# derekc22/UR3e

Measured on NVIDIA B200. Metric: env-steps/sec (UR3e+2F85, physics+controller), higher is better.
Workload: dtype f32

## Files before the change

ur3e_b200/csrc/batch_impl.cuh:

```cuda
#pragma once
#include <cstdio>
#include <cstdlib>
#include <cstring>
#include <limits>
#include <type_traits>
#include <vector>

#include "batch_base.h"
#include "compile_model.h"
#include "merge_bodies.h"
#include "env.cuh"
#include "query.cuh"
#include "query_fwd.cuh"
#include "render.cuh"
#include "rollout.h"

#ifndef UR3E_BLOCKS_PER_SM
#define UR3E_BLOCKS_PER_SM 2
#endif
#ifndef UR3E_LS_TOL
#define UR3E_LS_TOL 1e-2
#endif
#ifndef UR3E_MAX_WPB
#define UR3E_MAX_WPB 16
#endif

namespace ur3e {
enum Op { OP_STEP = 0, OP_RESET = 1, OP_SET_STATE = 2 };

template <typename Real>
struct KArgs {
  const DevModel<Real>* m;
  EnvCfg<Real> c;
  SolverOpts<Real> opt;
  const EnvCfg<Real>* c_dev; const SolverOpts<Real>* opt_dev;
  void* st;
  int* ovf_count; int* ovf_list;
  const int* list_count; const int* list;
  int lite_maxcon, lite_maxefc;
  int mid_maxcon, mid_maxefc;
  int* ovf2_count; int* ovf2_list;
  int* ovf_stat;
  int cap_con, cap_efc;
  long long n;
  int op;
  const Real* act; Real* obs; Real* rew; uint8_t* term; uint8_t* trunc; Real* final_obs;
  Real* sens;
  const uint8_t* mask;
  unsigned long long seed, env_base;
  const Real* qpos_in; const Real* qvel_in; const Real* ws_in;
};

template <typename Real, typename D> __host__ __device__ constexpr size_t arena_stride() { return (sizeof(Arena<Real, D>) + 15) / 16 * 16; }
template <typename Real, typename D> __host__ __device__ constexpr int warps_per_block() {
#ifdef UR3E_FORCE_WPB
  return UR3E_FORCE_WPB;
#endif
  int per_sm = (int)((233472 - 1024 * UR3E_BLOCKS_PER_SM) / arena_stride<Real, D>());
  int w = per_sm / UR3E_BLOCKS_PER_SM;
#ifdef UR3E_MID_MAX_WPB
  if (D::EXACT && D::MAXCON == 16 && w > UR3E_MID_MAX_WPB) w = UR3E_MID_MAX_WPB;
#endif
  return w > UR3E_MAX_WPB ? UR3E_MAX_WPB : (w < 1 ? 1 : w);
}

template <typename Real, typename D>
__global__ void __launch_bounds__(warps_per_block<Real, D>() * 32) env_kernel(const KArgs<Real> a) {
  constexpr int WPB = warps_per_block<Real, D>();
  extern __shared__ int4 smem_raw[];
  const int warp = threadIdx.x >> 5;
  const long long e = (long long)blockIdx.x * WPB + warp;
  if (e >= a.n) return;
  Arena<Real, D>& s = *reinterpret_cast<Arena<Real, D>*>(reinterpret_cast<unsigned char*>(smem_raw) + warp * arena_stride<Real, D>());
  const DevModel<Real>& m = *a.m;
  const EnvCfg<Real>& c = a.c;
  constexpr int NW = sizeof(EnvState<Real, D>) / 16;
  int4* gst = reinterpret_cast<int4*>(static_cast<EnvState<Real, D>*>(a.st) + e);
  int4* sst = reinterpret_cast<int4*>(&s.st);
  if (a.op == OP_RESET && a.mask && !a.mask[e]) return;
  WARP_FOR(i, NW) sst[i] = gst[i];
  IF_LANE0 { s.overflow = 0; s.ncon = 0; s.nefc = 0; s.solver_iter = 0; s.cap_con = D::MAXCON; s.cap_efc = D::MAXEFC; }
  WARP_SYNC();
  const int od = c.obs_dim;
  IF_LANE0 s.st.tier = 0;
  if (a.op == OP_RESET) {
    env_reset(m, c, s, a.opt, a.seed, a.env_base + (unsigned long long)e);
    ContactFlags cf = contact_flags(m, c, s);
    write_obs(m, c, s, cf);
    if (a.obs) { WARP_FOR(i, od) a.obs[e * od + i] = s.obs[i]; }
  } else if (a.op == OP_SET_STATE) {
    WARP_FOR(i, m.nq) s.st.qpos[i] = a.qpos_in[e * m.nq + i];
    WARP_FOR(i, m.nv) { s.st.qvel[i] = a.qvel_in[e * m.nv + i]; s.st.qacc_ws[i] = a.ws_in ? a.ws_in[e * m.nv + i] : Real(0); }
    WARP_SYNC();
    forward_cold(m, s, a.opt, false);
    update_cache(m, c, s);
  }
  WARP_SYNC();
  WARP_FOR(i, NW) gst[i] = sst[i];
}

constexpr int TIER_HOLD = 8;
template <typename Real, typename D, bool SENS = false>
__global__ void __launch_bounds__(warps_per_block<Real, D>() * 32, UR3E_BLOCKS_PER_SM) step_kernel(const KArgs<Real> a) {
  constexpr int WPB = warps_per_block<Real, D>();
  extern __shared__ int4 smem_raw[];
  const int warp = threadIdx.x >> 5;
  Arena<Real, D>& s = *reinterpret_cast<Arena<Real, D>*>(reinterpret_cast<unsigned char*>(smem_raw) + warp * arena_stride<Real, D>());
  const DevModel<Real>& m = *a.m;
  const EnvCfg<Real>& c = a.c;
  constexpr int NW = sizeof(EnvState<Real, D>) / 16;
  const int od = c.obs_dim;
  long long count = a.n; int iters = 1;
  if (a.list) { count = *a.list_count; const long long per = (long long)gridDim.x * WPB; iters = (int)((count + per - 1) / per); }
  for (int it = 0; it < iters; ++it) {
    const long long idx = ((long long)it * gridDim.x + blockIdx.x) * WPB + warp;
    if (idx >= count) return;
    const long long e = a.list ? (long long)a.list[idx] : idx;
    EnvState<Real, D>* const rec = static_cast<EnvState<Real, D>*>(a.st) + e;
    if (a.ovf_list && !a.list) {
      const int tier = rec->tier;
      if (tier & 0xff) {
        IF_LANE0 {
          if ((tier >> 8) && a.ovf2_list) { const int k = atomicAdd(a.ovf2_count, 1); a.ovf2_list[k] = (int)e; }
          else { const int k = atomicAdd(a.ovf_count, 1); a.ovf_list[k] = (int)e; }
        }
        return;
      }
    }
    int4* gst = reinterpret_cast<int4*>(rec);
    int4* sst = reinterpret_cast<int4*>(&s.st);
    WARP_FOR(i, NW) sst[i] = gst[i];
    IF_LANE0 {
      s.overflow = 0; s.ncon = 0; s.nefc = 0; s.solver_iter = 0;
      s.cap_con = (a.cap_con > 0 && a.cap_con < D::MAXCON) ? a.cap_con : D::MAXCON; s.cap_efc = (a.cap_efc > 0 && a.cap_efc < D::MAXEFC) ? a.cap_efc : D::MAXEFC;
    }
    WARP_SYNC();
    StepOut<Real> r = env_step(m, c, s, a.opt, a.act + e * c.act_dim, *a.opt_dev, SENS ? a.sens : nullptr, e);
    if (a.ovf_list && s.overflow) {
      IF_LANE0 { const int k = atomicAdd(a.ovf_count, 1); a.ovf_list[k] = (int)e; }
      continue;
    }
    if (a.lite_maxcon > 0) {
      IF_LANE0 {
        const bool big = s.max_ncon > a.lite_maxcon || s.max_nefc > a.lite_maxefc;
        const bool big2 = a.mid_maxcon > 0 && (s.max_ncon > a.mid_maxcon || s.max_nefc > a.mid_maxefc);
        const int h1 = s.st.tier & 0xff, h2 = s.st.tier >> 8;
        s.st.tier = (big ? TIER_HOLD : (h1 > 0 ? h1 - 1 : 0)) | ((big2 ? TIER_HOLD : (h2 > 0 ? h2 - 1 : 0)) << 8);
        if (big && a.ovf_stat) atomicAdd(a.ovf_stat, 1);
      }
    }
    const int done = r.terminated | r.truncated;
    if (done && a.final_obs) { WARP_FOR(i, od) a.final_obs[e * od + i] = s.obs[i]; }
    if (done && c.auto_reset) {
      env_reset(m, *a.c_dev, s, *a.opt_dev, a.seed, a.env_base + (unsigned long long)e);
      ContactFlags cf = contact_flags(m, c, s);
      write_obs(m, c, s, cf);
    }
    WARP_FOR(i, od) a.obs[e * od + i] = s.obs[i];
    IF_LANE0 { a.rew[e] = r.reward; a.term[e] = (uint8_t)r.terminated; a.trunc[e] = (uint8_t)r.truncated; }
    WARP_SYNC();
    WARP_FOR(i, NW) gst[i] = sst[i];
    WARP_SYNC();
  }
}

template <typename Real, typename D>
__global__ void state_io_kernel(EnvState<Real, D>* st, long long n, int nq, int nv, Real* qpos, Real* qvel, Real* ws) {
  long long i = (long long)blockIdx.x * blockDim.x + threadIdx.x;
  long long e = i / 64; int k = (int)(i % 64);
  if (e >= n) return;
  if (k < nq && qpos) qpos[e * nq + k] = st[e].qpos[k];
  if (k < nv && qvel) qvel[e * nv + k] = st[e].qvel[k];
  if (k < nv && ws) ws[e * nv + k] = st[e].qacc_ws[k];
}

template <typename Real, typename D>
__global__ void stats_kernel(EnvState<Real, D>* st, long long n, double* out, int reset) {
  long long e = (long long)blockIdx.x * blockDim.x + threadIdx.x;
  for (int k = 0; k < NSTAT; ++k) {
    double d = 0.0;
    if (e < n) { d = k == ST_RETURN ? (double)st[e].stat[k].f : (double)st[e].stat[k].i; if (reset) st[e].stat[k].i = 0; }
    for (int o = 16; o > 0; o >>= 1) d += __shfl_xor_sync(0xffffffffu, d, o);
    if ((threadIdx.x & 31) == 0 && d != 0.0) atomicAdd(out + k, d);
  }
}

template <typename Real, typename D>
__global__ void rollout_gather_kernel(const EnvState<Real, D>* src, long long n, const int* ids, EnvState<Real, D>* dst, long long m) {
  const long long j = ((long long)blockIdx.x * blockDim.x + threadIdx.x) >> 5;
  const int lane = threadIdx.x & 31;
  if (j >= m) return;
  constexpr int NW = sizeof(EnvState<Real, D>) / 16;
  const long long e = ids[j];
  int4* d = reinterpret_cast<int4*>(dst + j);
  const bool valid = e >= 0 && e < n;
  if (valid) {
    const int4* g = reinterpret_cast<const int4*>(src + e);
    for (int i = lane; i < NW; i += 32) d[i] = g[i];
  } else {
    for (int i = lane; i < NW; i += 32) d[i] = make_int4(0, 0, 0, 0);
  }
  __syncwarp();
  EnvState<Real, D>& r = dst[j];
  if (valid) {
    if (lane < NSTAT) r.stat[lane].i = 0;
  } else {
    const Real nan = std::numeric_limits<Real>::quiet_NaN();
    for (int i = lane; i < D::NQ; i += 32) r.qpos[i] = nan;
    for (int i = lane; i < D::NV; i += 32) { r.qvel[i] = nan; r.qacc_ws[i] = nan; }
    for (int i = lane; i < CACHE_SIZE; i += 32) r.cache[i] = nan;
  }
}

template <typename Real, typename D>
// ... 29 lines not shown
  WARP_SYNC();
  const long long k = a.k;
  query_env(m, s, a.q, a.k, a.pos ? a.pos + e * k * 3 : nullptr, a.mat ? a.mat + e * k * 9 : nullptr, a.vel ? a.vel + e * k * 6 : nullptr, a.local);
}

template <typename Real, typename D>
struct QJArgs {
  const DevModel<Real>* m;
  const EnvState<Real, D>* st;
  const QueryEntry<Real>* q; int k;
  long long n;
  Real *jacp, *jacr, *M, *bias;
};

template <typename Real, typename D>
__global__ void __launch_bounds__(warps_per_block<Real, QueryDims<D>>() * 32) query_jac_kernel(const QJArgs<Real, D> a) {
  using DK = QueryDims<D>;
  constexpr int WPB = warps_per_block<Real, DK>();
  extern __shared__ int4 smem_raw[];
  const int warp = threadIdx.x >> 5;
  const long long e = (long long)blockIdx.x * WPB + warp;
  if (e >= a.n) return;
  Arena<Real, DK>& s = *reinterpret_cast<Arena<Real, DK>*>(reinterpret_cast<unsigned char*>(smem_raw) + warp * arena_stride<Real, DK>());
  const DevModel<Real>& m = *a.m;
  const EnvState<Real, D>& rec = a.st[e];
  WARP_FOR(i, m.nq) s.st.qpos[i] = rec.qpos[i];
  if (a.M || a.bias) { WARP_FOR(i, m.nv) s.st.qvel[i] = rec.qvel[i]; }
  WARP_SYNC();
  const long long nv = m.nv, kj = (long long)a.k * 3 * nv;
  query_jac_env(m, s, a.q, a.k, a.jacp ? a.jacp + e * kj : nullptr, a.jacr ? a.jacr + e * kj : nullptr, a.M ? a.M + e * nv * nv : nullptr,
                a.bias ? a.bias + e * nv : nullptr);
}

template <typename Real, typename D>
struct QFArgs {
  const DevModel<Real>* m;
  const EnvState<Real, D>* st;
  SolverOpts<Real> opt;
  long long n;
  const Real* ctrl;
  FwdOut<Real> o;
};

template <typename Real, typename D>
__global__ void __launch_bounds__(warps_per_block<Real, D>() * 32, 1) query_fwd_kernel(const QFArgs<Real, D> a) {
  constexpr int WPB = warps_per_block<Real, D>();
  constexpr long long C = D::HAS_CONTACT ? D::MAXCON : 0;
  extern __shared__ int4 smem_raw[];
  const int warp = threadIdx.x >> 5;
  const long long e = (long long)blockIdx.x * WPB + warp;
  if (e >= a.n) return;
  Arena<Real, D>& s = *reinterpret_cast<Arena<Real, D>*>(reinterpret_cast<unsigned char*>(smem_raw) + warp * arena_stride<Real, D>());
  const DevModel<Real>& m = *a.m;
  constexpr int NW = sizeof(EnvState<Real, D>) / 16;
  const int4* gst = reinterpret_cast<const int4*>(a.st + e);
  int4* sst = reinterpret_cast<int4*>(&s.st);
  WARP_FOR(i, NW) sst[i] = gst[i];
  const long long nv = m.nv;
  FwdOut<Real> o;
  o.qacc = a.o.qacc ? a.o.qacc + e * nv : nullptr;
  o.qfrc_constraint = a.o.qfrc_constraint ? a.o.qfrc_constraint + e * nv : nullptr;
  o.info = a.o.info ? a.o.info + e * 4 : nullptr;
  o.contact_geom = a.o.contact_geom ? a.o.contact_geom + e * C * 2 : nullptr;
  o.contact_dist = a.o.contact_dist ? a.o.contact_dist + e * C : nullptr;
  o.contact_pos = a.o.contact_pos ? a.o.contact_pos + e * C * 3 : nullptr;
  o.contact_frame = a.o.contact_frame ? a.o.contact_frame + e * C * 9 : nullptr;
  o.contact_force = a.o.contact_force ? a.o.contact_force + e * C * 6 : nullptr;
  o.flags = a.o.flags ? a.o.flags + e : nullptr;
  o.sensordata = a.o.sensordata ? a.o.sensordata + e * NSENSOR : nullptr;
  forward_query_env(m, s, a.opt, a.ctrl ? a.ctrl + e * m.nu : nullptr, o);
}

template <typename Real, typename D>
struct RPArgs {
  const DevModel<Real>* m;
  const EnvState<Real, D>* st;
  const QueryEntry<Real>* q; int k;
  long long n, count;
  const int* env_ids;
  Real* pose;
};

template <typename Real, typename D>
__global__ void __launch_bounds__(warps_per_block<Real, QueryDims<D>>() * 32) render_pose_kernel(const RPArgs<Real, D> a) {
  using DK = QueryDims<D>;
  constexpr int WPB = warps_per_block<Real, DK>();
  extern __shared__ int4 smem_raw[];
  const int warp = threadIdx.x >> 5;
  const long long i = (long long)blockIdx.x * WPB + warp;
  if (i >= a.count) return;
  const long long e = a.env_ids ? (long long)a.env_ids[i] : i;
  if (e < 0 || e >= a.n) return;
  Arena<Real, DK>& s = *reinterpret_cast<Arena<Real, DK>*>(reinterpret_cast<unsigned char*>(smem_raw) + warp * arena_stride<Real, DK>());
  const DevModel<Real>& m = *a.m;
  const EnvState<Real, D>& rec = a.st[e];
  WARP_FOR(j, m.nq) s.st.qpos[j] = rec.qpos[j];
  WARP_SYNC();
  render_pose_env(m, s, a.q, a.k, a.pose + i * 12 * (a.k + 1));
}

template <typename Real>
struct RArgs {
  const RenderGeom<Real>* geoms; int k;
  RenderCam<Real> cam;
  const Real* pose;
  const int* env_ids; long long n;
  unsigned char* rgb; Real* depth; int* seg;
};

constexpr int RENDER_THREADS = 256, RENDER_TILE = 1024;
// ... 493 lines not shown
```

ur3e_b200/csrc/engine.cuh:

```cuda
#pragma once
#include "dev_model.h"
#include "warp_model.cuh"

namespace ur3e {

template <int NB_, int NV_, int NQ_, int NU_, int NG_, int NPAIR_, int MAXCON_, int MAXEFC_, int SPLIT_ = NV_, bool EXACT_ = false>
struct Dims {
  static constexpr bool EXACT = EXACT_;
  static constexpr int SPLIT = SPLIT_;
  static constexpr int NB = NB_, NV = NV_, NQ = NQ_, NU = NU_, NG = NG_ > 0 ? NG_ : 1, NPAIR = NPAIR_ > 0 ? NPAIR_ : 1;
  static constexpr int MAXCON = MAXCON_ > 0 ? MAXCON_ : 1, MAXEFC = MAXEFC_ > 0 ? MAXEFC_ : 1;
  static constexpr bool HAS_CONTACT = MAXCON_ > 0;
  static constexpr int NS = MAXSITE;
  static constexpr int ACT_CAP = MAXCON_ <= 8 ? 16 : (MAXCON_ <= 16 ? 20 : 24);
  static constexpr int MAXACT = !HAS_CONTACT ? 1 : (NPAIR < ACT_CAP ? NPAIR : ACT_CAP);
  static constexpr int NGRP = MAXEQ + (NPAIR < MAXCON ? NPAIR : MAXCON);
  static constexpr int MAXCONNECT = 2;
  static constexpr int MAXDENSE = HAS_CONTACT ? 3 * MAXCONNECT + 3 * MAXCON : 1;
};
using DimsRaw = Dims<8, 6, 6, 6, 1, 0, 0, 12>;
using DimsGrip = Dims<17, 14, 14, 7, 6, 12, 12, 56>;
using DimsGripExact = Dims<17, 14, 14, 7, 6, 12, 12, 56, 14, true>;
using DimsMain = Dims<19, 20, 21, 7, 14, 48, 24, 92, 14>;
using DimsMainLite = Dims<19, 20, 21, 7, 14, 48, 8, 44, 14, true>;
using DimsMainMid = Dims<19, 20, 21, 7, 14, 48, 16, 68, 14, true>;

constexpr int STAGE_PTS = 8;
constexpr int STAGE_W = 3 + 4 * STAGE_PTS;

enum RowType { ROW_EQ = 0, ROW_EQJ = 1, ROW_FRICTION = 2, ROW_LIMIT_LO = 3, ROW_LIMIT_HI = 4, ROW_CON_N = 5, ROW_CON_T1 = 6, ROW_CON_T2 = 7 };

constexpr int NSTAT = 16;
constexpr int MAX_FRAME_SKIP = 256;
enum StatSlot { ST_EPISODES = 0, ST_RETURN, ST_LENGTH, ST_SUCCESS, ST_TERM_REACH, ST_TERM_TOPPLE, ST_TERM_COLLISION, ST_TRUNC, ST_UNSTABLE,
                ST_NEFC, ST_NCON, ST_ITER, ST_SUBSTEPS, ST_OVERFLOW,
                ST_PADCON , ST_STEPS  };
template <typename Real, typename D>
struct alignas(16) EnvState {
  Real qpos[D::NQ], qvel[D::NV], qacc_ws[D::NV];
  Real cache[CACHE_SIZE];
  Real ep_return;
  union { int i; float f; } stat[NSTAT];
  int t, episode;
  int tier;
};

#ifdef UR3E_CANARY
#define UR3E_GUARD(n) unsigned guard##n;
constexpr unsigned CANARY_WORD = 0xC0FFEE5Au;
#else
#define UR3E_GUARD(n)
#endif

template <typename Real, typename D>
struct Arena {
  EnvState<Real, D> st;
  UR3E_GUARD(0)
  Real qacc[D::NV], ctrl[D::NU], act_force[D::NU];
  Real xpos[D::NB][3];
  union alignas(8) {
    struct { Real xmat[D::NB][9], xipos[D::NB][3]; } k;
    struct { Real H[(D::NV + 1) * (D::NV + 2) / 2]; } n;
  } fr;
  union { alignas(16) Real colbuf[1][32]; Real obs[32]; };
  Real cdof[D::NV][6];
  UR3E_GUARD(1)
  alignas(8) Real M[D::NV * (D::NV + 1) / 2];
  UR3E_GUARD(2)
  Real qfrc_smooth[D::NV], qfrc_bias[D::NV], qfrc_constraint[D::NV], grad[D::NV], search[D::NV], Ma[D::NV];
  union { Real Mv[D::NV]; Real dinv[D::NV]; };
  Real site_xpos[D::NS][3], site_xmat[1][9] , site_velp[D::NS][3];
  Real con_pos[D::MAXCON][3], con_dist[D::MAXCON], con_mu[D::MAXCON];
  union {
    Real frame[D::MAXCON][9];
    Real gpos[D::NG][3];
  } cu;
  static_assert(D::MAXCON * 9 >= D::NG * 3 || !D::HAS_CONTACT, "geom positions alias the contact frames");
  Real efc_aref[D::MAXEFC], efc_D[D::MAXEFC], efc_jv[D::MAXEFC], efc_Dact[D::MAXEFC];
  UR3E_GUARD(3)
  Real efc_force[D::MAXEFC], efc_jar[D::MAXEFC];
  UR3E_GUARD(4)
  uint8_t con_pair[D::MAXCON], con_row[D::MAXCON];
  uint8_t efc_type[D::MAXEFC], efc_id[D::MAXEFC];
  int grp_mask[D::NGRP];
  uint8_t grp_row0[D::NGRP], grp_nrow[D::NGRP];
  uint8_t stage_n[D::MAXACT], stage_off[D::MAXACT], act_pair[D::MAXACT];
  Real eqj_deriv[MAXEQ];
  uint8_t sp_fl[D::NV], sp_lo[D::NV], sp_hi[D::NV], sp_ej[D::NV];
  int lim_lo, lim_hi;
  short nd, rf0, rl0;
  short ncon, nefc, ne, nf, nl, ngrp, overflow, solver_iter, bad, max_ncon, max_nefc, cap_con, cap_efc;
  short sum_ncon, sum_nefc, sum_iter, warn;
  short coupled;
  UR3E_GUARD(5)
  union alignas(16) {
    struct { Real cinert[D::NB][10], cdof_dot[D::NV][6], cvel[D::NB][6], cfrc[D::NB][6]; } dyn;
    struct { Real lmat[D::NB][9], lpos[D::NB][3]; } kin;
    Real stage[D::MAXACT][STAGE_W];
    Real efc_J[D::MAXDENSE][D::NV];
  } u;
  UR3E_GUARD(6)
};

#ifdef UR3E_CANARY
template <typename Real, typename D> UR3E_HD void canary_set(Arena<Real, D>& s) {
  IF_LANE0 { s.guard0 = s.guard1 = s.guard2 = s.guard3 = s.guard4 = s.guard5 = s.guard6 = CANARY_WORD; }
}
template <typename Real, typename D> UR3E_HD int canary_bad(const Arena<Real, D>& s) {
  return (s.guard0 != CANARY_WORD) | ((s.guard1 != CANARY_WORD) << 1) | ((s.guard2 != CANARY_WORD) << 2) | ((s.guard3 != CANARY_WORD) << 3) |
         ((s.guard4 != CANARY_WORD) << 4) | ((s.guard5 != CANARY_WORD) << 5) | ((s.guard6 != CANARY_WORD) << 6);
}
#endif

template <typename D> struct StaticModel { static constexpr int NLEVEL = 0, NM = 0, NFL = 0, NEQ = 0, NSITE = 0, NDEQ = 0, NEJ = 0; static constexpr bool DAMPING = false; };
template <> struct StaticModel<DimsGripExact> { static constexpr int NLEVEL = 10, NM = 81, NFL = 6, NEQ = 3, NSITE = 1, NDEQ = 6, NEJ = 1; static constexpr bool DAMPING = true; };
template <> struct StaticModel<DimsMainLite> { static constexpr int NLEVEL = 10, NM = 102, NFL = 6, NEQ = 3, NSITE = 4, NDEQ = 6, NEJ = 1; static constexpr bool DAMPING = true; };
template <> struct StaticModel<DimsMainMid> : StaticModel<DimsMainLite> {};
#define UR3E_MODEL_CONST(fn, STATIC, field) \
  template <typename D, typename Real> UR3E_HD auto fn(const DevModel<Real>& m) { if constexpr (D::EXACT) return StaticModel<D>::STATIC; else return m.field; }
UR3E_MODEL_CONST(nlevel_, NLEVEL, nlevel) UR3E_MODEL_CONST(nM_, NM, nM) UR3E_MODEL_CONST(nfl_, NFL, nfl) UR3E_MODEL_CONST(neq_, NEQ, neq)
UR3E_MODEL_CONST(nsite_, NSITE, nsite) UR3E_MODEL_CONST(ndeq_, NDEQ, ndeq) UR3E_MODEL_CONST(nej_, NEJ, nej)
template <typename D, typename Real> UR3E_HD bool has_damping_(const DevModel<Real>& m) { if constexpr (D::EXACT) return StaticModel<D>::DAMPING; else return m.has_damping != 0; }
template <typename D, typename Real> UR3E_HD int split_(const DevModel<Real>& m) { if constexpr (D::EXACT) return D::SPLIT; else return m.split; }

template <typename D, typename Real> UR3E_HD int nv_(const DevModel<Real>& m) { if constexpr (D::EXACT) return D::NV; else return m.nv; }
template <typename D, typename Real> UR3E_HD int nb_(const DevModel<Real>& m) { if constexpr (D::EXACT) return D::NB; else return m.nbody; }
template <typename D, typename Real> UR3E_HD int nq_(const DevModel<Real>& m) { if constexpr (D::EXACT) return D::NQ; else return m.nq; }
template <typename D, typename Real> UR3E_HD int nu_(const DevModel<Real>& m) { if constexpr (D::EXACT) return D::NU; else return m.nu; }
template <typename D, typename Real> UR3E_HD int ng_(const DevModel<Real>& m) { if constexpr (D::EXACT) return D::NG; else return m.ngeom; }
template <typename D, typename Real> UR3E_HD int np_(const DevModel<Real>& m) { if constexpr (D::EXACT) return D::NPAIR; else return m.npair; }

template <typename Real> struct Num;
template <> struct Num<float> {
  static UR3E_HD float sqrt(float x) { return ::sqrtf(x); }
  static UR3E_HD float sin(float x) { return ::sinf(x); }
  static UR3E_HD void sincos(float x, float* sn, float* cs) {
    float q = ::rintf(x * 0.636619772f);
    int n = (int)q;
    float r = ::fmaf(q, -1.5707963109016418f, x); r = ::fmaf(q, -1.5893254712295857e-8f, r);
    float r2 = r * r;
    float sp = r + r * r2 * (-1.6666654611e-1f + r2 * (8.3321608736e-3f + r2 * -1.9515295891e-4f));
    float cp = 1.0f + r2 * (-0.5f + r2 * (4.166664568298827e-2f + r2 * (-1.388731625493765e-3f + r2 * 2.443315711809948e-5f)));
    float s0 = (n & 1) ? cp : sp, c0 = (n & 1) ? sp : cp;
    *sn = (n & 2) ? -s0 : s0;
    *cs = ((n + 1) & 2) ? -c0 : c0;
  }
  static UR3E_HD float cos(float x) { return ::cosf(x); }
  static UR3E_HD float atan2(float y, float x) { return ::atan2f(y, x); }
  static UR3E_HD float pow(float x, float y) { return ::powf(x, y); }
#if defined(__CUDA_ARCH__)
  static UR3E_HD float pow_pos(float x, float y) { return x > 0 ? __powf(x, y) : 0.f; }
#else
// ... 1335 lines not shown
```

ur3e_b200/csrc/env.cuh:

```cuda
#pragma once
#include "engine.cuh"

namespace ur3e {

UR3E_HD void philox4x32(uint32_t c0, uint32_t c1, uint32_t c2, uint32_t c3, uint32_t k0, uint32_t k1, uint32_t* out) {
  for (int r = 0; r < 10; ++r) {
    uint64_t p0 = (uint64_t)0xD2511F53u * c0, p1 = (uint64_t)0xCD9E8D57u * c2;
    uint32_t n0 = (uint32_t)(p1 >> 32) ^ c1 ^ k0, n1 = (uint32_t)p1, n2 = (uint32_t)(p0 >> 32) ^ c3 ^ k1, n3 = (uint32_t)p0;
    c0 = n0; c1 = n1; c2 = n2; c3 = n3; k0 += 0x9E3779B9u; k1 += 0xBB67AE85u;
  }
  out[0] = c0; out[1] = c1; out[2] = c2; out[3] = c3;
}
template <typename Real> UR3E_HD Real u01(uint32_t x) { return (Real)((double)x * (1.0 / 4294967296.0)); }

template <typename Real> UR3E_HD void rot_err(const Real* xmat, const Real* rv, Real* err) {
  Real ang = Num<Real>::sqrt(dot3(rv, rv)), q[4] = {1, 0, 0, 0};
  if (ang > Real(1e-30)) { Real sn, cs; Num<Real>::sincos(ang * Real(0.5), &sn, &cs); sn /= ang; q[0] = cs; q[1] = rv[0] * sn; q[2] = rv[1] * sn; q[3] = rv[2] * sn; }
  Real Rt[9], E[9]; quat2mat(Rt, q);
  for (int i = 0; i < 3; ++i) for (int j = 0; j < 3; ++j) E[3 * i + j] = Rt[3 * i] * xmat[3 * j] + Rt[3 * i + 1] * xmat[3 * j + 1] + Rt[3 * i + 2] * xmat[3 * j + 2];
  Real tr = E[0] + E[4] + E[8], w, x, y, z;
  if (tr > 0) { Real s = Num<Real>::sqrt(tr + 1) * 2; w = Real(0.25) * s; x = (E[7] - E[5]) / s; y = (E[2] - E[6]) / s; z = (E[3] - E[1]) / s; }
  else if (E[0] > E[4] && E[0] > E[8]) { Real s = Num<Real>::sqrt(1 + E[0] - E[4] - E[8]) * 2; w = (E[7] - E[5]) / s; x = Real(0.25) * s; y = (E[1] + E[3]) / s; z = (E[2] + E[6]) / s; }
  else if (E[4] > E[8]) { Real s = Num<Real>::sqrt(1 + E[4] - E[0] - E[8]) * 2; w = (E[2] - E[6]) / s; x = (E[1] + E[3]) / s; y = Real(0.25) * s; z = (E[5] + E[7]) / s; }
  else { Real s = Num<Real>::sqrt(1 + E[8] - E[0] - E[4]) * 2; w = (E[3] - E[1]) / s; x = (E[2] + E[6]) / s; y = (E[5] + E[7]) / s; z = Real(0.25) * s; }
  Real nq = Num<Real>::sqrt(w * w + x * x + y * y + z * z); w /= nq; x /= nq; y /= nq; z /= nq;
  if (w < 0) { w = -w; x = -x; y = -y; z = -z; }
  Real sn = Num<Real>::sqrt(x * x + y * y + z * z), a = 2 * Num<Real>::atan2(sn, w);
  Real k = sn < Real(1e-12) ? Real(2) : a / sn;
  err[0] = k * x; err[1] = k * y; err[2] = k * z;
}

template <typename Real, typename D>
UR3E_HD void update_cache(const DevModel<Real>& m, const EnvCfg<Real>& c, Arena<Real, D>& s) {
  int site = c.site_tcp;
  if (site < 0) return;
  int b = m.site_body[site];
  WARP_FOR(i, CACHE_SIZE) {
    Real v;
    if (i < 3) v = s.site_xpos[site][i];
    else if (i < 12) v = s.site_xmat[0][i - 3];
    else if (i < 48) {
      int r = (i - 12) / 6, k = (i - 12) - 6 * r;
      if (r < 3) { Real col[3]; jac_col(m, s, k, s.site_xpos[site], b, col); v = col[r]; }
      else v = ((m.body_dofmask[b] >> k) & 1u) ? s.cdof[k][r - 3] : Real(0);
    } else v = s.qfrc_bias[i - 48];
    s.st.cache[i] = v;
  }
  WARP_SYNC();
}

template <typename Real, typename D>
UR3E_HD void pid_task(const DevModel<Real>& m, const EnvCfg<Real>& c, Arena<Real, D>& s, const Real* traj) {
  const Real* ch = s.st.cache;
  Real e[6], F[6];
  for (int k = 0; k < 3; ++k) e[k] = traj[k] - ch[k];
  rot_err(ch + 3, traj + 3, e + 3);
  for (int r = 0; r < 6; ++r) {
    Real v = 0; for (int k = 0; k < 6; ++k) v += ch[12 + 6 * r + k] * s.st.qvel[k];
    int g = r < 3 ? r : 3 + r;
    F[r] = c.gains[g] * e[r] - c.gains[g + 3] * v;
  }
  WARP_FOR(k, 6) { Real v = ch[48 + k]; for (int r = 0; r < 6; ++r) v += ch[12 + 6 * r + k] * F[r]; s.ctrl[k] = v; }
  IF_LANE0 s.ctrl[nu_<D>(m) - 1] = traj[6] * m.act_ctrlrange[nu_<D>(m) - 1][1];
}

template <typename Real, typename D>
UR3E_HD void controller(const DevModel<Real>& m, const EnvCfg<Real>& c, Arena<Real, D>& s, const Real* act) {
  switch (c.ctrl_mode) {
    case CTRL_RAW: { WARP_FOR(a, nu_<D>(m)) s.ctrl[a] = act[a]; break; }
    case CTRL_PD_JOINT: {
      WARP_FOR(i, 6) {
        Real q = s.st.qpos[i], tq = q + (act[i] - q);
        tq = rmin(rmax(tq, m.dof_range[i][0]), m.dof_range[i][1]);
        Real u = c.gains[i] * (tq - q) + c.gains[6 + i] * -s.st.qvel[i];
        s.ctrl[i] = rmin(rmax(u, m.act_ctrlrange[i][0]), m.act_ctrlrange[i][1]);
      }
      if (nu_<D>(m) > 6) { IF_LANE0 s.ctrl[nu_<D>(m) - 1] = act[6] * m.act_ctrlrange[nu_<D>(m) - 1][1]; }
      break;
    }
    case CTRL_PID_TASK: { Real traj[7]; for (int k = 0; k < 7; ++k) traj[k] = act[k]; pid_task(m, c, s, traj); break; }
    case CTRL_PID_TASK_ENV: {
      Real traj[7] = {act[0], act[1], act[2], c.tool_rotvec[0], c.tool_rotvec[1], c.tool_rotvec[2], act[3]};
      pid_task(m, c, s, traj); break;
    }
    case CTRL_PINV: {
      const Real* ch = s.st.cache;
      Real e[6], y[6];
      for (int k = 0; k < 3; ++k) e[k] = act[k] - ch[k];
      { Real rv[3] = {act[3], act[4], act[5]}; rot_err(ch + 3, rv, e + 3); }
      for (int blk = 0; blk < 2; ++blk) {
        const Real* J = ch + 12 + 18 * blk;
        Real A[6];
        int idx = 0;
        for (int r = 0; r < 3; ++r) for (int c2 = r; c2 < 3; ++c2) { Real v = 0; for (int k = 0; k < 6; ++k) v += J[6 * r + k] * J[6 * c2 + k]; A[idx++] = v; }
        const Real c00 = A[3] * A[5] - A[4] * A[4], c01 = A[2] * A[4] - A[1] * A[5], c02 = A[1] * A[4] - A[2] * A[3];
        const Real det = A[0] * c00 + A[1] * c01 + A[2] * c02, id = Real(1) / det;
        const Real c11 = A[0] * A[5] - A[2] * A[2], c12 = A[1] * A[2] - A[0] * A[4], c22 = A[0] * A[3] - A[1] * A[1];
        const Real* b = e + 3 * blk;
        y[3 * blk + 0] = (c00 * b[0] + c01 * b[1] + c02 * b[2]) * id;
        y[3 * blk + 1] = (c01 * b[0] + c11 * b[1] + c12 * b[2]) * id;
        y[3 * blk + 2] = (c02 * b[0] + c12 * b[1] + c22 * b[2]) * id;
      }
      WARP_FOR(i, 6) {
        const Real q = s.st.qpos[i], qd = s.st.qvel[i];
        Real u = 0;
        for (int blk = 0; blk < 2; ++blk) {
          const Real* J = ch + 12 + 18 * blk;
          const Real dth = J[i] * y[3 * blk] + J[6 + i] * y[3 * blk + 1] + J[12 + i] * y[3 * blk + 2];
          Real tq = rmin(rmax(q + dth, m.dof_range[i][0]), m.dof_range[i][1]);
          Real ub = c.gains[12 * blk + i] * (tq - q) + c.gains[12 * blk + 6 + i] * -qd;
          u += rmin(rmax(ub, m.act_ctrlrange[i][0]), m.act_ctrlrange[i][1]);
        }
        s.ctrl[i] = u;
      }
      if (nu_<D>(m) > 6) { IF_LANE0 s.ctrl[nu_<D>(m) - 1] = act[6] * m.act_ctrlrange[nu_<D>(m) - 1][1]; }
      break;
    }
    default: break;
  }
  WARP_SYNC();
}

struct ContactFlags { int grasp_count; int table_hit; int self_hit; };

template <typename Real, typename D>
UR3E_HD int contact_bits(const DevModel<Real>& m, const Arena<Real, D>& s) {
  int f = 0;
  if constexpr (D::HAS_CONTACT) {
    WARP_FOR(k, s.ncon) {
      const int p = s.con_pair[k], f1 = m.geom_flags[m.pair_g1[p]], f2 = m.geom_flags[m.pair_g2[p]], any = f1 | f2;
      if ((any & GF_MUG) && (any & GF_LPAD)) f |= 1;
      if ((any & GF_MUG) && (any & GF_RPAD)) f |= 2;
      if (((f1 & GF_TABLE) && (f2 & GF_GRIPPER)) || ((f2 & GF_TABLE) && (f1 & GF_GRIPPER))) f |= 4;
      if ((f1 & GF_ARM) && (f2 & GF_ARM) && !((f1 & GF_GRIPPER) && (f2 & GF_GRIPPER))) f |= 8;
    }
  }
  return warp_or(f);
}

// ... 24 lines not shown
        o[23] = robust ? Real(1) : Real(0);
      } else if (c.obs_kind == OBS_V0) {
        o[9] = (Real)cf.grasp_count;
        for (int k = 0; k < 3; ++k) o[10 + k] = s.site_xpos[c.site_pad][k];
      } else {
        o[9] = (Real)cf.grasp_count;
        for (int k = 0; k < 3; ++k) o[10 + k] = s.site_velp[c.site_tcp][k];
      }
    }
  }
  WARP_SYNC();
}

template <typename Real> UR3E_HD Real norm3(Real a, Real b, Real c) { return Num<Real>::sqrt(a * a + b * b + c * c); }

template <typename Real> UR3E_HD Real reward_v2(const Real* o, Real grip) {
  Real mug_z = o[5], gx = o[9], gy = o[10], gz = o[11], grasped = o[23];
  Real xy = Num<Real>::sqrt(gx * gx + gy * gy), zerr = Num<Real>::abs(gz - Real(0.02)), place = norm3(o[12], o[13], o[14]);
  Real ready = Num<Real>::exp(-10 * xy) * Num<Real>::exp(-20 * zerr);
  Real r = Real(2) * ready + Real(2) * grip * ready + Real(10) * grasped * ready;
  r += Real(8) * grasped * Num<Real>::tanh(Real(8) * rmax(Real(0), mug_z));
  r += grasped * (Real(4) * Num<Real>::exp(-15 * place) - Real(1.5) * place);
  if (grasped != 0 && place < Real(0.05)) r += Real(50);
  r += Real(-1) * rmax(Real(0), -gz);
  r += Real(-0.01) * norm3(o[15], o[16], o[17]);
  return r;
}

template <typename Real> UR3E_HD Real reward_v0(const Real* o, Real grip, Real half_h, int table_hit, int toppled, int self_hit) {
  Real gs = o[9];
  Real top = o[5] + half_h, bot = o[5] - half_h, pad_top = o[12] - top, g2c = o[2] - o[5];
  Real hx = o[0] - o[3], hy = o[1] - o[4], herr = Num<Real>::sqrt(hx * hx + hy * hy);
  bool valid = gs == 2 && Num<Real>::abs(pad_top) < Real(0.04) && herr < Real(0.03);
  Real height_error = g2c - Real(0.5), z_tol = Real(0.1);
  Real descent = (1 / z_tol) * (height_error + z_tol) * Num<Real>::exp(-(1 / z_tol) * height_error);
  Real ready = Num<Real>::exp(-herr * herr) * Num<Real>::exp(-pad_top * pad_top) * Num<Real>::exp(-height_error * height_error) * 100 * Num<Real>::exp(-grip * grip);
  Real align = 4 * Num<Real>::exp(-60 * herr * herr);
  Real g1 = gs >= 1 ? Real(1) : Real(0), g2 = gs == 2 ? Real(1) : Real(0);
  Real grasp = Real(5.5) * g1 + Real(8.5) * g2 + Real(23.5) * grip * ready + Real(28.5) * g2 * ready + Real(11.5) * g2 * ready * Num<Real>::tanh(8 * grip);
  Real lift = 12 * g2 * Num<Real>::tanh(4 * bot);
  Real dplace = norm3(o[3] - o[6], o[4] - o[7], o[5] - o[8]);
  Real placement = -2 * dplace + 20 * Num<Real>::exp(-70 * dplace * dplace);
  if (dplace < Real(0.05) && valid) placement += 40;
  Real dh = o[5] - o[2] + Real(0.5);
  Real danger = rmin(Real(0), Real(-100000000000.0) * dh * dh * dh);
  Real pen = Real(-40) * self_hit + Real(-25) * table_hit + Real(-8) * toppled + Real(-4) * rmax(Real(0), pad_top) + danger;
  Real action_r = Real(700.5) * grip * ready, bonus = Real(1700.5) * g2 * ready * Num<Real>::tanh(10 * grip);
  return descent + align + grasp + lift + placement + action_r + bonus + pen;
}

template <typename Real> struct StepOut { Real reward; int terminated, truncated, reason; };

template <typename Real, typename D>
UR3E_HD StepOut<Real> reward_done(const DevModel<Real>& m, const EnvCfg<Real>& c, Arena<Real, D>& s, const ContactFlags& cf, const Real* act) {
  StepOut<Real> r; r.reward = 0; r.terminated = 0; r.truncated = 0; r.reason = 0;
  const Real* o = s.obs;
  int t = s.st.t;
  if (c.term_kind == TERM_V2) {
    r.reward = reward_v2(o, act[c.act_dim - 1]);
    t += 1;
    Real dpick = norm3(o[0] - o[3], o[1] - o[4], o[2] - o[5]);
    int toppled = o[5] <= c.topple_z;
    if (dpick > 1) { r.terminated = 1; r.reason = ST_TERM_REACH; }
    else if (cf.self_hit) { r.terminated = 1; r.reason = ST_TERM_COLLISION; }
    else if (toppled) { r.terminated = 1; r.reason = ST_TERM_TOPPLE; }
    if (t >= c.max_steps) r.truncated = 1;
    if (norm3(o[3] - o[6], o[4] - o[7], o[5] - o[8]) < Real(0.05)) { r.terminated = 1; r.reward += 50; r.reason = ST_SUCCESS; }
  } else if (c.term_kind == TERM_V0) {
    int toppled = o[5] <= c.topple_z;
    r.reward = reward_v0(o, act[c.act_dim - 1], c.mug_size[2], cf.table_hit, toppled, cf.self_hit);
    Real dpick = norm3(o[0] - o[3], o[1] - o[4], o[2] - o[5]), dplace = norm3(o[3] - o[6], o[4] - o[7], o[5] - o[8]);
    if (dplace < Real(0.005)) { r.terminated = 1; r.reason = ST_SUCCESS; }
    else if (dpick > 1) { r.terminated = 1; r.reason = ST_TERM_REACH; }
    else if (cf.self_hit) { r.terminated = 1; r.reason = ST_TERM_COLLISION; }
    else if (toppled) { r.terminated = 1; r.reason = ST_TERM_TOPPLE; }
    if (t >= c.max_steps) r.truncated = 1;
    t += 1;
  } else {
    r.reward = c.reward_kind == REW_MINUS1 ? Real(-1) : Real(0);
    if (c.max_steps > 0 && t >= c.max_steps) r.truncated = 1;
    t += 1;
  }
  IF_LANE0 s.st.t = t;
  return r;
}

template <typename Real, typename D>
UR3E_PHASE void env_reset(const DevModel<Real>& m, const EnvCfg<Real>& c, Arena<Real, D>& s, const SolverOpts<Real>& opt, uint64_t seed, uint64_t env_id) {
  int key = c.reset_key;
  WARP_FOR(i, nq_<D>(m)) s.st.qpos[i] = key >= 0 ? m.key_qpos[key][i] : m.qpos0[i];
  WARP_FOR(i, nv_<D>(m)) { s.st.qvel[i] = key >= 0 ? m.key_qvel[key][i] : Real(0); s.st.qacc_ws[i] = 0; s.qacc[i] = 0; }
  WARP_FOR(i, nu_<D>(m)) s.ctrl[i] = 0;
  WARP_SYNC();
  if (c.reset_noise != NOISE_NONE && c.body_mug >= 0) {
    uint32_t r[4];
    philox4x32((uint32_t)env_id, (uint32_t)(env_id >> 32), (uint32_t)s.st.episode, 0u, (uint32_t)seed, (uint32_t)(seed >> 32), r);
    Real ylo = c.reset_noise == NOISE_HIGH ? Real(-0.25) : c.reset_noise == NOISE_MED ? Real(-0.2) : Real(-0.1);
    Real yhi = c.reset_noise == NOISE_HIGH ? Real(0.2) : c.reset_noise == NOISE_MED ? Real(0.1) : Real(0.01);
    IF_LANE0 { int qa = m.body_qadr[c.body_mug]; s.st.qpos[qa] += Real(0.02) * u01<Real>(r[0]); s.st.qpos[qa + 1] += ylo + (yhi - ylo) * u01<Real>(r[1]); }
  }
  IF_LANE0 { s.st.t = 0; s.st.ep_return = 0; s.st.episode += 1; }
  WARP_SYNC();
  forward_cold(m, s, opt, false);
  update_cache(m, c, s);
}

template <typename Real, typename D>
UR3E_HD StepOut<Real> env_step(const DevModel<Real>& m, const EnvCfg<Real>& c, Arena<Real, D>& s, const SolverOpts<Real>& opt, const Real* act,
                               const SolverOpts<Real>& opt_cold, Real* sens_base = nullptr, long long env = 0) {
  IF_LANE0 { s.overflow = 0; }
#ifdef UR3E_CANARY
  canary_set(s);
#endif
  controller(m, c, s, act);
  IF_LANE0 { s.max_ncon = 0; s.max_nefc = 0; s.sum_ncon = 0; s.sum_nefc = 0; s.sum_iter = 0; s.warn = 0; }
  for (int k = 0; k < c.frame_skip; ++k) {
    const int w = substep(m, s, opt, opt_cold, k == c.frame_skip - 1 ? sens_base : nullptr, env);
    IF_LANE0 {
      s.warn |= w; s.sum_nefc += s.nefc; s.sum_ncon += s.ncon; s.sum_iter += s.solver_iter;
      if (s.ncon > s.max_ncon) s.max_ncon = s.ncon;
      if (s.nefc > s.max_nefc) s.max_nefc = s.nefc;
    }
  }
  WARP_SYNC();
#ifdef UR3E_CANARY
  { const int bad = canary_bad(s); if (bad) { IF_LANE0 { printf("ur3e_b200: arena guard word clobbered (mask 0x%x, env %lld)\n", bad, env); s.warn |= 8; } } }
#endif
  const int warn = s.warn;
  const int sn = s.sum_nefc, sc = s.sum_ncon, si = s.sum_iter;
  update_cache(m, c, s);
  ContactFlags cf = contact_flags(m, c, s);
  write_obs(m, c, s, cf);
  StepOut<Real> r = reward_done(m, c, s, cf, act);
  IF_LANE0 {
    s.st.ep_return += r.reward;
    auto* st = s.st.stat;
    st[ST_NEFC].i += sn; st[ST_NCON].i += sc; st[ST_ITER].i += si; st[ST_SUBSTEPS].i += c.frame_skip;
    if (warn) st[ST_UNSTABLE].i += 1;
    if (s.overflow) st[ST_OVERFLOW].i += 1;
    st[ST_STEPS].i += 1;
    if (cf.grasp_count > 0) st[ST_PADCON].i += 1;
    if (r.terminated || r.truncated) {
      st[ST_EPISODES].i += 1; st[ST_RETURN].f += (float)s.st.ep_return; st[ST_LENGTH].i += s.st.t;
      if (r.terminated && r.reason) st[r.reason].i += 1;
      if (r.truncated && !r.terminated) st[ST_TRUNC].i += 1;
    }
  }
  WARP_SYNC();
  return r;
}

}
```

Measured before the change: 27.44 million.

## Shrink per-warp shared arena to sim state; keep cache and bookkeeping in global

```diff
diff --git a/ur3e_b200/csrc/batch_impl.cuh b/ur3e_b200/csrc/batch_impl.cuh
--- a/ur3e_b200/csrc/batch_impl.cuh
+++ b/ur3e_b200/csrc/batch_impl.cuh
@@ -23,6 +23,9 @@
 #endif
 #ifndef UR3E_MAX_WPB
 #define UR3E_MAX_WPB 16
+#endif
+#ifndef UR3E_CONTACT_MAX_WPB
+#define UR3E_CONTACT_MAX_WPB 14
 #endif
 
 namespace ur3e {
@@ -61,7 +64,21 @@
 #ifdef UR3E_MID_MAX_WPB
   if (D::EXACT && D::MAXCON == 16 && w > UR3E_MID_MAX_WPB) w = UR3E_MID_MAX_WPB;
 #endif
-  return w > UR3E_MAX_WPB ? UR3E_MAX_WPB : (w < 1 ? 1 : w);
+  const int cap = D::HAS_CONTACT ? UR3E_CONTACT_MAX_WPB : UR3E_MAX_WPB;
+  return w > cap ? cap : (w < 1 ? 1 : w);
+}
+
+template <typename Real, typename D>
+__device__ __forceinline__ void load_sim(Arena<Real, D>& s, const EnvState<Real, D>* rec) {
+  using Rec = EnvState<Real, D>;
+  static_assert(offsetof(Rec, cache) == sizeof(Real) * (D::NQ + 2 * D::NV), "SimState is the first part of the record");
+  const int4* g = reinterpret_cast<const int4*>(rec); int4* w = reinterpret_cast<int4*>(&s.st);
+  WARP_FOR(i, (int)(sizeof(SimState<Real, D>) / 16)) w[i] = g[i];
+}
+template <typename Real, typename D>
+__device__ __forceinline__ void store_sim(EnvState<Real, D>* rec, const Arena<Real, D>& s) {
+  Real* g = reinterpret_cast<Real*>(rec); const Real* v = reinterpret_cast<const Real*>(&s.st);
+  WARP_FOR(i, D::NQ + 2 * D::NV) g[i] = v[i];
 }
 
 template <typename Real, typename D>
@@ -74,17 +91,15 @@
   Arena<Real, D>& s = *reinterpret_cast<Arena<Real, D>*>(reinterpret_cast<unsigned char*>(smem_raw) + warp * arena_stride<Real, D>());
   const DevModel<Real>& m = *a.m;
   const EnvCfg<Real>& c = a.c;
-  constexpr int NW = sizeof(EnvState<Real, D>) / 16;
-  int4* gst = reinterpret_cast<int4*>(static_cast<EnvState<Real, D>*>(a.st) + e);
-  int4* sst = reinterpret_cast<int4*>(&s.st);
+  EnvState<Real, D>* const rec = static_cast<EnvState<Real, D>*>(a.st) + e;
   if (a.op == OP_RESET && a.mask && !a.mask[e]) return;
-  WARP_FOR(i, NW) sst[i] = gst[i];
+  load_sim(s, rec);
   IF_LANE0 { s.overflow = 0; s.ncon = 0; s.nefc = 0; s.solver_iter = 0; s.cap_con = D::MAXCON; s.cap_efc = D::MAXEFC; }
   WARP_SYNC();
   const int od = c.obs_dim;
-  IF_LANE0 s.st.tier = 0;
+  IF_LANE0 rec->tier = 0;
   if (a.op == OP_RESET) {
-    env_reset(m, c, s, a.opt, a.seed, a.env_base + (unsigned long long)e);
+    env_reset(m, c, s, *rec, a.opt, a.seed, a.env_base + (unsigned long long)e);
     ContactFlags cf = contact_flags(m, c, s);
     write_obs(m, c, s, cf);
     if (a.obs) { WARP_FOR(i, od) a.obs[e * od + i] = s.obs[i]; }
@@ -93,10 +108,10 @@
     WARP_FOR(i, m.nv) { s.st.qvel[i] = a.qvel_in[e * m.nv + i]; s.st.qacc_ws[i] = a.ws_in ? a.ws_in[e * m.nv + i] : Real(0); }
     WARP_SYNC();
     forward_cold(m, s, a.opt, false);
-    update_cache(m, c, s);
+    update_cache(m, c, s, rec->cache);
   }
   WARP_SYNC();
-  WARP_FOR(i, NW) gst[i] = sst[i];
+  store_sim(rec, s);
 }
 
 constexpr int TIER_HOLD = 8;
@@ -108,7 +123,6 @@
   Arena<Real, D>& s = *reinterpret_cast<Arena<Real, D>*>(reinterpret_cast<unsigned char*>(smem_raw) + warp * arena_stride<Real, D>());
   const DevModel<Real>& m = *a.m;
   const EnvCfg<Real>& c = a.c;
-  constexpr int NW = sizeof(EnvState<Real, D>) / 16;
   const int od = c.obs_dim;
   long long count = a.n; int iters = 1;
   if (a.list) { count = *a.list_count; const long long per = (long long)gridDim.x * WPB; iters = (int)((count + per - 1) / per); }
@@ -127,15 +141,13 @@
         return;
       }
     }
-    int4* gst = reinterpret_cast<int4*>(rec);
-    int4* sst = reinterpret_cast<int4*>(&s.st);
-    WARP_FOR(i, NW) sst[i] = gst[i];
+    load_sim(s, rec);
     IF_LANE0 {
       s.overflow = 0; s.ncon = 0; s.nefc = 0; s.solver_iter = 0;
       s.cap_con = (a.cap_con > 0 && a.cap_con < D::MAXCON) ? a.cap_con : D::MAXCON; s.cap_efc = (a.cap_efc > 0 && a.cap_efc < D::MAXEFC) ? a.cap_efc : D::MAXEFC;
     }
     WARP_SYNC();
-    StepOut<Real> r = env_step(m, c, s, a.opt, a.act + e * c.act_dim, *a.opt_dev, SENS ? a.sens : nullptr, e);
+    StepOut<Real> r = env_step(m, c, s, *rec, a.opt, a.act + e * c.act_dim, *a.opt_dev, a.ovf_list != nullptr, SENS ? a.sens : nullptr, e);
     if (a.ovf_list && s.overflow) {
       IF_LANE0 { const int k = atomicAdd(a.ovf_count, 1); a.ovf_list[k] = (int)e; }
       continue;
@@ -144,22 +156,22 @@
       IF_LANE0 {
         const bool big = s.max_ncon > a.lite_maxcon || s.max_nefc > a.lite_maxefc;
         const bool big2 = a.mid_maxcon > 0 && (s.max_ncon > a.mid_maxcon || s.max_nefc > a.mid_maxefc);
-        const int h1 = s.st.tier & 0xff, h2 = s.st.tier >> 8;
-        s.st.tier = (big ? TIER_HOLD : (h1 > 0 ? h1 - 1 : 0)) | ((big2 ? TIER_HOLD : (h2 > 0 ? h2 - 1 : 0)) << 8);
+        const int tier = rec->tier, h1 = tier & 0xff, h2 = tier >> 8;
+        rec->tier = (big ? TIER_HOLD : (h1 > 0 ? h1 - 1 : 0)) | ((big2 ? TIER_HOLD : (h2 > 0 ? h2 - 1 : 0)) << 8);
         if (big && a.ovf_stat) atomicAdd(a.ovf_stat, 1);
       }
     }
     const int done = r.terminated | r.truncated;
     if (done && a.final_obs) { WARP_FOR(i, od) a.final_obs[e * od + i] = s.obs[i]; }
     if (done && c.auto_reset) {
-      env_reset(m, *a.c_dev, s, *a.opt_dev, a.seed, a.env_base + (unsigned long long)e);
+      env_reset(m, *a.c_dev, s, *rec, *a.opt_dev, a.seed, a.env_base + (unsigned long long)e);
       ContactFlags cf = contact_flags(m, c, s);
       write_obs(m, c, s, cf);
     }
     WARP_FOR(i, od) a.obs[e * od + i] = s.obs[i];
     IF_LANE0 { a.rew[e] = r.reward; a.term[e] = (uint8_t)r.terminated; a.trunc[e] = (uint8_t)r.truncated; }
     WARP_SYNC();
-    WARP_FOR(i, NW) gst[i] = sst[i];
+    store_sim(rec, s);
     WARP_SYNC();
   }
 }
@@ -295,10 +307,7 @@
   if (e >= a.n) return;
   Arena<Real, D>& s = *reinterpret_cast<Arena<Real, D>*>(reinterpret_cast<unsigned char*>(smem_raw) + warp * arena_stride<Real, D>());
   const DevModel<Real>& m = *a.m;
-  constexpr int NW = sizeof(EnvState<Real, D>) / 16;
-  const int4* gst = reinterpret_cast<const int4*>(a.st + e);
-  int4* sst = reinterpret_cast<int4*>(&s.st);
-  WARP_FOR(i, NW) sst[i] = gst[i];
+  load_sim(s, a.st + e);
   const long long nv = m.nv;
   FwdOut<Real> o;
   o.qacc = a.o.qacc ? a.o.qacc + e * nv : nullptr;
diff --git a/ur3e_b200/csrc/engine.cuh b/ur3e_b200/csrc/engine.cuh
--- a/ur3e_b200/csrc/engine.cuh
+++ b/ur3e_b200/csrc/engine.cuh
@@ -44,6 +44,8 @@
   int t, episode;
   int tier;
 };
+template <typename Real, typename D>
+struct alignas(16) SimState { Real qpos[D::NQ], qvel[D::NV], qacc_ws[D::NV]; };
 
 #ifdef UR3E_CANARY
 #define UR3E_GUARD(n) unsigned guard##n;
@@ -54,7 +56,7 @@
 
 template <typename Real, typename D>
 struct Arena {
-  EnvState<Real, D> st;
+  SimState<Real, D> st;
   UR3E_GUARD(0)
   Real qacc[D::NV], ctrl[D::NU], act_force[D::NU];
   Real xpos[D::NB][3];
@@ -98,6 +100,7 @@
     struct { Real lmat[D::NB][9], lpos[D::NB][3]; } kin;
     Real stage[D::MAXACT][STAGE_W];
     Real efc_J[D::MAXDENSE][D::NV];
+    Real cache[CACHE_SIZE];
   } u;
   UR3E_GUARD(6)
 };
diff --git a/ur3e_b200/csrc/env.cuh b/ur3e_b200/csrc/env.cuh
--- a/ur3e_b200/csrc/env.cuh
+++ b/ur3e_b200/csrc/env.cuh
@@ -31,7 +31,7 @@
 }
 
 template <typename Real, typename D>
-UR3E_HD void update_cache(const DevModel<Real>& m, const EnvCfg<Real>& c, Arena<Real, D>& s) {
+UR3E_HD void update_cache(const DevModel<Real>& m, const EnvCfg<Real>& c, Arena<Real, D>& s, Real* out) {
   int site = c.site_tcp;
   if (site < 0) return;
   int b = m.site_body[site];
@@ -44,14 +44,15 @@
       if (r < 3) { Real col[3]; jac_col(m, s, k, s.site_xpos[site], b, col); v = col[r]; }
       else v = ((m.body_dofmask[b] >> k) & 1u) ? s.cdof[k][r - 3] : Real(0);
     } else v = s.qfrc_bias[i - 48];
-    s.st.cache[i] = v;
-  }
-  WARP_SYNC();
+    s.u.cache[i] = v;
+  }
+  WARP_SYNC();
+  WARP_FOR(i, CACHE_SIZE) out[i] = s.u.cache[i];
 }
 
 template <typename Real, typename D>
 UR3E_HD void pid_task(const DevModel<Real>& m, const EnvCfg<Real>& c, Arena<Real, D>& s, const Real* traj) {
-  const Real* ch = s.st.cache;
+  const Real* ch = s.u.cache;
   Real e[6], F[6];
   for (int k = 0; k < 3; ++k) e[k] = traj[k] - ch[k];
   rot_err(ch + 3, traj + 3, e + 3);
@@ -84,7 +85,7 @@
       pid_task(m, c, s, traj); break;
     }
     case CTRL_PINV: {
-      const Real* ch = s.st.cache;
+      const Real* ch = s.u.cache;
       Real e[6], y[6];
       for (int k = 0; k < 3; ++k) e[k] = act[k] - ch[k];
       { Real rv[3] = {act[3], act[4], act[5]}; rot_err(ch + 3, rv, e + 3); }
@@ -215,10 +216,10 @@
 template <typename Real> struct StepOut { Real reward; int terminated, truncated, reason; };
 
 template <typename Real, typename D>
-UR3E_HD StepOut<Real> reward_done(const DevModel<Real>& m, const EnvCfg<Real>& c, Arena<Real, D>& s, const ContactFlags& cf, const Real* act) {
+UR3E_HD StepOut<Real> reward_done(const DevModel<Real>& m, const EnvCfg<Real>& c, Arena<Real, D>& s, EnvState<Real, D>& rec, const ContactFlags& cf, const Real* act) {
   StepOut<Real> r; r.reward = 0; r.terminated = 0; r.truncated = 0; r.reason = 0;
   const Real* o = s.obs;
-  int t = s.st.t;
+  int t = rec.t;
   if (c.term_kind == TERM_V2) {
     r.reward = reward_v2(o, act[c.act_dim - 1]);
     t += 1;
@@ -244,12 +245,13 @@
     if (c.max_steps > 0 && t >= c.max_steps) r.truncated = 1;
     t += 1;
   }
-  IF_LANE0 s.st.t = t;
+  IF_LANE0 rec.t = t;
   return r;
 }
 
 template <typename Real, typename D>
-UR3E_PHASE void env_reset(const DevModel<Real>& m, const EnvCfg<Real>& c, Arena<Real, D>& s, const SolverOpts<Real>& opt, uint64_t seed, uint64_t env_id) {
+UR3E_PHASE void env_reset(const DevModel<Real>& m, const EnvCfg<Real>& c, Arena<Real, D>& s, EnvState<Real, D>& rec, const SolverOpts<Real>& opt, uint64_t seed,
+                          uint64_t env_id) {
   int key = c.reset_key;
   WARP_FOR(i, nq_<D>(m)) s.st.qpos[i] = key >= 0 ? m.key_qpos[key][i] : m.qpos0[i];
   WARP_FOR(i, nv_<D>(m)) { s.st.qvel[i] = key >= 0 ? m.key_qvel[key][i] : Real(0); s.st.qacc_ws[i] = 0; s.qacc[i] = 0; }
@@ -257,24 +259,26 @@
   WARP_SYNC();
   if (c.reset_noise != NOISE_NONE && c.body_mug >= 0) {
     uint32_t r[4];
-    philox4x32((uint32_t)env_id, (uint32_t)(env_id >> 32), (uint32_t)s.st.episode, 0u, (uint32_t)seed, (uint32_t)(seed >> 32), r);
+    philox4x32((uint32_t)env_id, (uint32_t)(env_id >> 32), (uint32_t)rec.episode, 0u, (uint32_t)seed, (uint32_t)(seed >> 32), r);
     Real ylo = c.reset_noise == NOISE_HIGH ? Real(-0.25) : c.reset_noise == NOISE_MED ? Real(-0.2) : Real(-0.1);
     Real yhi = c.reset_noise == NOISE_HIGH ? Real(0.2) : c.reset_noise == NOISE_MED ? Real(0.1) : Real(0.01);
     IF_LANE0 { int qa = m.body_qadr[c.body_mug]; s.st.qpos[qa] += Real(0.02) * u01<Real>(r[0]); s.st.qpos[qa + 1] += ylo + (yhi - ylo) * u01<Real>(r[1]); }
   }
-  IF_LANE0 { s.st.t = 0; s.st.ep_return = 0; s.st.episode += 1; }
+  IF_LANE0 { rec.t = 0; rec.ep_return = 0; rec.episode += 1; }
   WARP_SYNC();
   forward_cold(m, s, opt, false);
-  update_cache(m, c, s);
-}
-
-template <typename Real, typename D>
-UR3E_HD StepOut<Real> env_step(const DevModel<Real>& m, const EnvCfg<Real>& c, Arena<Real, D>& s, const SolverOpts<Real>& opt, const Real* act,
-                               const SolverOpts<Real>& opt_cold, Real* sens_base = nullptr, long long env = 0) {
+  update_cache(m, c, s, rec.cache);
+}
+
+template <typename Real, typename D>
+UR3E_HD StepOut<Real> env_step(const DevModel<Real>& m, const EnvCfg<Real>& c, Arena<Real, D>& s, EnvState<Real, D>& rec, const SolverOpts<Real>& opt,
+                               const Real* act, const SolverOpts<Real>& opt_cold, bool handoff, Real* sens_base = nullptr, long long env = 0) {
   IF_LANE0 { s.overflow = 0; }
 #ifdef UR3E_CANARY
   canary_set(s);
 #endif
+  WARP_FOR(i, CACHE_SIZE) s.u.cache[i] = rec.cache[i];
+  WARP_SYNC();
   controller(m, c, s, act);
   IF_LANE0 { s.max_ncon = 0; s.max_nefc = 0; s.sum_ncon = 0; s.sum_nefc = 0; s.sum_iter = 0; s.warn = 0; }
   for (int k = 0; k < c.frame_skip; ++k) {
@@ -289,22 +293,23 @@
 #ifdef UR3E_CANARY
   { const int bad = canary_bad(s); if (bad) { IF_LANE0 { printf("ur3e_b200: arena guard word clobbered (mask 0x%x, env %lld)\n", bad, env); s.warn |= 8; } } }
 #endif
+  if (handoff && s.overflow) { StepOut<Real> r; r.reward = 0; r.terminated = 0; r.truncated = 0; r.reason = 0; return r; }
   const int warn = s.warn;
   const int sn = s.sum_nefc, sc = s.sum_ncon, si = s.sum_iter;
-  update_cache(m, c, s);
+  update_cache(m, c, s, rec.cache);
   ContactFlags cf = contact_flags(m, c, s);
   write_obs(m, c, s, cf);
-  StepOut<Real> r = reward_done(m, c, s, cf, act);
+  StepOut<Real> r = reward_done(m, c, s, rec, cf, act);
   IF_LANE0 {
-    s.st.ep_return += r.reward;
-    auto* st = s.st.stat;
+    rec.ep_return += r.reward;
+    auto* st = rec.stat;
     st[ST_NEFC].i += sn; st[ST_NCON].i += sc; st[ST_ITER].i += si; st[ST_SUBSTEPS].i += c.frame_skip;
     if (warn) st[ST_UNSTABLE].i += 1;
     if (s.overflow) st[ST_OVERFLOW].i += 1;
     st[ST_STEPS].i += 1;
     if (cf.grasp_count > 0) st[ST_PADCON].i += 1;
     if (r.terminated || r.truncated) {
-      st[ST_EPISODES].i += 1; st[ST_RETURN].f += (float)s.st.ep_return; st[ST_LENGTH].i += s.st.t;
+      st[ST_EPISODES].i += 1; st[ST_RETURN].f += (float)rec.ep_return; st[ST_LENGTH].i += rec.t;
       if (r.terminated && r.reason) st[r.reason].i += 1;
       if (r.truncated && !r.terminated) st[ST_TRUNC].i += 1;
     }
```

Result: no change. 27.41 million, median of 6 (-0.1%).
